# meilisearch/arroy

Measured on NVIDIA H100. Metric: index-build vectors/sec, higher is better.
Workload: dtype f32

## Files before the change

### arroy_b200/csrc/arroy_b200.cu

```cuda
#include <cuda_runtime.h>

#include <algorithm>
#include <atomic>
#include <chrono>
#include <cstdio>
#include <cstdlib>
#include <cstring>
#include <mutex>
#include <stdexcept>
#include <string>
#include <thread>
#include <vector>

#include "../../include/arroy_b200.h"
#include "build.cuh"
#include "search.cuh"
#include <cublas_v2.h>

#include "xrerank.cuh"
#include "tcgemm.cuh"
#include "frerank.cuh"

using namespace ab;

// ... 355 lines not shown
    W.active.ensure(4);
    W.error.ensure(4);
    W.keys.ensure(32ull * tw);
    size_t ws_bytes = (size_t)WS_VECS * ld * 4;
    int use_smem = ws_bytes <= 200 * 1024 ? 1 : 0;
    if (!use_smem) W.scratch.ensure(ws_bytes * tw);
    const int spec = (use_smem && (size_t)WS_VECS_SPEC * ld * 4 <= 200 * 1024 && !(getenv("ARROY_B200_SPEC") && atoi(getenv("ARROY_B200_SPEC")) == 0)) ? 1 : 0;
    if (spec) ws_bytes = (size_t)WS_VECS_SPEC * ld * 4;

    BuildParams P{};
    P.items = c->items.as<float>(); P.ih0 = c->h0.as<float>(); P.ih1 = c->h1.as<float>();
    P.n = (uint32_t)n; P.d = c->dim; P.ld = ld; P.metric = c->metric; P.K = K; P.n_trees = tw;
    P.st = W.st.as<TreeState>(); P.frames = W.frames.as<Frame>(); P.recs = W.recs.as<Record>(); P.rec_cap = rec_cap;
    P.perm[0] = W.perm0.as<uint32_t>(); P.perm[1] = W.perm1.as<uint32_t>();
    P.flags = W.flags.as<uint8_t>(); P.unit_left = W.unit_left.as<uint32_t>(); P.units_per_tree = units;
    P.pool = W.pool.as<float>(); P.pool_stride = pool_stride; P.pool_cap = pool_cap; P.pool_counter = W.pool_counter.as<uint32_t>();
    P.jobs = W.jobs.as<Job>(); P.scratch = W.scratch.as<float>(); P.use_smem_ws = use_smem; P.spec = spec;
    P.active = W.active.as<uint32_t>(); P.error = W.error.as<int32_t>();
    P.sub_rows = nullptr; P.sub_off = nullptr;
    P.lat_mask = getenv("ARROY_B200_LATMASK") ? (uint32_t)atoi(getenv("ARROY_B200_LATMASK")) : 3u;
    P.small_max = getenv("ARROY_B200_SMALL_MAX") ? (uint32_t)atoi(getenv("ARROY_B200_SMALL_MAX")) : (uint32_t)std::max<uint64_t>(2048, (6ull << 20) / (4ull * ld));
    P.max_inner = 1024u;
    P.timing = nullptr;
    if (getenv("ARROY_B200_CTRL_TIMING")) { W.timing.ensure(24 * 8); CK(cudaMemsetAsync(W.timing.p, 0, 24 * 8, c->stream)); P.timing = W.timing.as<unsigned long long>(); }
    if (sub.rows) {
        const uint64_t b = sub.off[t0], e = sub.off[t0 + tw];
        std::vector<uint64_t> off(tw + 1);
        for (uint32_t t = 0; t <= tw; ++t) off[t] = sub.off[t0 + t] - b;
        W.sub_rows.ensure(std::max<size_t>(16, 4ull * (e - b)));
        W.sub_off.ensure(8ull * (tw + 1));
        if (e > b) CK(cudaMemcpyAsync(W.sub_rows.p, sub.rows + b, 4ull * (e - b), cudaMemcpyHostToDevice, c->stream));
        CK(cudaMemcpy(W.sub_off.p, off.data(), 8ull * (tw + 1), cudaMemcpyHostToDevice));
        P.sub_rows = W.sub_rows.as<uint32_t>(); P.sub_off = W.sub_off.as<uint64_t>();
    }

    std::vector<uint32_t> keys((size_t)tw * 8);
    for (uint32_t t = 0; t < tw; ++t)
        for (int i = 0; i < 8; ++i) {
            const uint8_t* s = seeds[t0 + t] + 4 * i;
            keys[(size_t)t * 8 + i] = (uint32_t)s[0] | ((uint32_t)s[1] << 8) | ((uint32_t)s[2] << 16) | ((uint32_t)s[3] << 24);
        }
    CK(cudaMemcpyAsync(W.keys.p, keys.data(), keys.size() * 4, cudaMemcpyHostToDevice, c->stream));
    CK(cudaMemsetAsync(W.pool_counter.p, 0, 4, c->stream));
    CK(cudaMemsetAsync(W.error.p, 0, 4, c->stream));
    CK(cudaMemcpyAsync(W.active.p, &tw, 4, cudaMemcpyHostToDevice, c->stream));
    const uint64_t* d_start = nullptr;
    if (sub.start_pos) {
// ... 66 lines not shown
            P.shadow_small_chunk = getenv("ARROY_B200_SHADOW_CHUNK") ? (uint32_t)std::min(4, std::max(1, atoi(getenv("ARROY_B200_SHADOW_CHUNK")))) : 4u;
            P.shadow_big_units = getenv("ARROY_B200_SHADOW_BIG") ? (uint32_t)atoi(getenv("ARROY_B200_SHADOW_BIG")) : 512u;
            P.shadow_big_chunk = getenv("ARROY_B200_SHADOW_BIGCHUNK") ? (uint32_t)std::max(4, atoi(getenv("ARROY_B200_SHADOW_BIGCHUNK"))) : 8u;
        }
    }
    if (persist) {
        W.slots.ensure(sizeof(PSlot) * tw);
        W.abort.ensure(4);
        CK(cudaMemsetAsync(W.slots.p, 0, sizeof(PSlot) * tw, c->stream));
        CK(cudaMemsetAsync(W.abort.p, 0, 4, c->stream));
        W.cur_normal.ensure(4ull * pool_stride * tw);
        P.slots = W.slots.as<PSlot>();
        P.cur_normal = W.cur_normal.as<float>();
        P.abort = W.abort.as<int>();
        const char* rf = getenv("ARROY_B200_ROOT_FUSE");
        P.root_fused = (!sub.rows && tw >= 2 && P.d >= 32 && (size_t)ROOT_TB * ld * 4 <= psmem && !(rf && atoi(rf) == 0)) ? 1 : 0;
        W.root.ensure(8);
        CK(cudaMemsetAsync(W.root.p, 0, 8, c->stream));
        P.root_ready = W.root.as<uint32_t>(); P.root_ticket = W.root.as<uint32_t>() + 1;
    }

    auto launch_step = [&](cudaStream_t s) {
        launch_control(ctrl1, tw, 1, ctrl_smem, s, P, 0u);
        if (P.planes.hi) work_kernel_shadow<<<c->sm_count * 2, WORK_THREADS, wsmem + perm_smem, s>>>(P.jobs, (int)tw, P.items, P.planes, P.ih0, P.d, P.ld, P.metric, P.shadow_min_units, P.shadow_stats);
        else work_kernel<<<work_grid, WORK_THREADS, wsmem, s>>>(P.jobs, (int)tw, P.items, P.ih0, P.d, P.ld, P.metric, interleave);
    };
    auto launch_tree_step = [&](uint32_t t, cudaStream_t s) {
        launch_control(ctrlc, 1, cluster, ctrl_smem, s, P, t);
        if (P.planes.hi) work_kernel_shadow<<<tree_grid, WORK_THREADS, wsmem1 + perm_smem, s>>>(P.jobs + t, 1, P.items, P.planes, P.ih0, P.d, P.ld, P.metric, P.shadow_min_units, P.shadow_stats);
        else work_kernel<<<tree_grid, WORK_THREADS, wsmem1, s>>>(P.jobs + t, 1, P.items, P.ih0, P.d, P.ld, P.metric, 0);
    };
    if (!lockstep) {
        while (c->tree_streams.size() < tw) { cudaStream_t st; CK(cudaStreamCreateWithFlags(&st, cudaStreamNonBlocking)); c->tree_streams.push_back(st); }
        while (c->tree_events.size() < (size_t)tw + 1) { cudaEvent_t ev; CK(cudaEventCreateWithFlags(&ev, cudaEventDisableTiming)); c->tree_events.push_back(ev); }
    }

    CK(cudaStreamSynchronize(c->stream));
    c->breakdown[0] += ms_since(t_setup);
    auto t_graph = std::chrono::steady_clock::now();
    cudaGraphExec_t gexec = nullptr;
    if (use_graph && !persist) {
        std::vector<uint8_t> key(sizeof(BuildParams) + 16);
        memcpy(key.data(), &P, sizeof(BuildParams));
        int32_t sched[4] = {(lockstep ? 1 : 0) | (interleave << 1) | (cluster << 8), steps_per_batch, (int32_t)tw, (int32_t)ctrl_smem};
        memcpy(key.data() + sizeof(BuildParams), sched, 16);
        if (c->cached_exec && key == c->cached_graph_key) gexec = c->cached_exec;
        else {
            if (c->cached_exec) { cudaGraphExecDestroy(c->cached_exec); c->cached_exec = nullptr; }
            if (c->cached_graph) { cudaGraphDestroy(c->cached_graph); c->cached_graph = nullptr; }
            c->cached_graph_key.clear();
            cudaGraph_t graph = nullptr;
            CK(cudaStreamBeginCapture(c->stream, cudaStreamCaptureModeThreadLocal));
// ... 53 lines not shown
            }
        }
        CK(cudaMemcpyAsync((void*)h_active, W.active.p, 4, cudaMemcpyDeviceToHost, c->stream));
        CK(cudaMemcpyAsync((void*)h_error, W.error.p, 4, cudaMemcpyDeviceToHost, c->stream));
        CK(cudaStreamSynchronize(c->stream));
        steps = 1;
        c->n_launches += 1;
        { float kms = 0; CK(cudaEventElapsedTime(&kms, c->ev_p0, c->ev_p1)); c->stats[5] += kms; }
        if (*h_error != ERR_NONE) {
            const int e = *h_error;
            if (e == ERR_ABORT) throw Cancelled("The corresponding build process has been cancelled");
            if (e == ERR_HANG) throw std::runtime_error("forest build made no progress (persistent schedule watchdog)");
            throw CapacityError(e == ERR_DEPTH ? "tree deeper than MAX_DEPTH frames" : e == ERR_RECORDS ? "node record table overflow" : "normal pool overflow");
        }
        if (*h_active != 0) throw std::runtime_error("forest build ended with unfinished trees (internal state machine error)");
    } else
    for (;;) {
        if (steps > max_steps) throw std::runtime_error("forest build did not converge (internal state machine error)");
        if (use_graph) CK(cudaGraphLaunch(gexec, c->stream));
        else if (profile) {
            for (int i = 0; i < steps_per_batch; ++i) {
                launch_control(ctrl1, tw, 1, ctrl_smem, c->stream, P, 0u);
                CK(cudaEventRecord(pev[2 * i], c->stream));
                if (P.planes.hi) work_kernel_shadow<<<c->sm_count * 2, WORK_THREADS, wsmem + perm_smem, c->stream>>>(P.jobs, (int)tw, P.items, P.planes, P.ih0, P.d, P.ld, P.metric, P.shadow_min_units, P.shadow_stats);
                else work_kernel<<<work_grid, WORK_THREADS, wsmem, c->stream>>>(P.jobs, (int)tw, P.items, P.ih0, P.d, P.ld, P.metric, interleave);
                CK(cudaEventRecord(pev[2 * i + 1], c->stream));
            }
            CK(cudaStreamSynchronize(c->stream));
            for (int i = 0; i < steps_per_batch; ++i) {
                float ms = 0; CK(cudaEventElapsedTime(&ms, pev[2 * i], pev[2 * i + 1])); c->stats[5] += ms;
                if (getenv("ARROY_B200_TRACE") && steps + i < 48) fprintf(stderr, "[trace] step %llu work_kernel %.3f ms\n", (unsigned long long)(steps + i), ms);
            }
        }
        else if (lockstep) { for (int i = 0; i < steps_per_batch; ++i) launch_step(c->stream); CK(cudaGetLastError()); }
        else {
            CK(cudaEventRecord(c->tree_events[0], c->stream));
            for (uint32_t t = 0; t < tw; ++t) {
                cudaStream_t st = c->tree_streams[t];
                CK(cudaStreamWaitEvent(st, c->tree_events[0], 0));
                for (int i = 0; i < steps_per_batch; ++i) launch_tree_step(t, st);
                CK(cudaEventRecord(c->tree_events[1 + t], st));
                CK(cudaStreamWaitEvent(c->stream, c->tree_events[1 + t], 0));
            }
            CK(cudaGetLastError());
        }
        steps += steps_per_batch;
        c->n_launches += 2ull * steps_per_batch * (lockstep ? 1 : tw);
        CK(cudaMemcpyAsync((void*)h_active, W.active.p, 4, cudaMemcpyDeviceToHost, c->stream));
        CK(cudaMemcpyAsync((void*)h_error, W.error.p, 4, cudaMemcpyDeviceToHost, c->stream));
        CK(cudaStreamSynchronize(c->stream));
        if (*h_error != ERR_NONE) {
            int e = *h_error;
            throw CapacityError(e == ERR_DEPTH ? "tree deeper than MAX_DEPTH frames" : e == ERR_RECORDS ? "node record table overflow" : "normal pool overflow");
        }
        if (*h_active == 0) break;
        if (cancel && cancel(cancel_arg)) throw Cancelled("The corresponding build process has been cancelled");
    }
    c->stats[1] += (double)steps;
    c->breakdown[2] += ms_since(t_loop);
    if (P.timing) {
        unsigned long long tv[24]; CK(cudaMemcpy(tv, P.timing, sizeof(tv), cudaMemcpyDeviceToHost));
        const char* nm[20] = {"decide", "rng", "gather", "norms", "two_means_rest", "finish_split", "cluster_scan", "prefix", "partition", "attempts", "inner", "total", "tm_dot_rest", "tm_update", "tm_dots", "tm_finish", "tm_recurrence", "publish_fence", "recur_it0", "recur_it1_9"};
        const double att = (double)std::max<unsigned long long>(tv[9], 1);
        fprintf(stderr, "[ctrl timing] attempts %llu, in-cluster %llu; cycles per attempt:", tv[9], tv[10]);
        for (int i = 0; i < 20; ++i) if (i != 9 && i != 10) fprintf(stderr, " %s %.0f", nm[i], (double)tv[i] / att);
        if (tv[20]) fprintf(stderr, "; fused root pass: %llu cycles on the slowest worker", tv[20]);
        fprintf(stderr, "\n");
    }
    c->breakdown[5] += (double)(steps / steps_per_batch);
    auto t_d2h = std::chrono::steady_clock::now();

    W.final_ids.ensure(4ull * n * tw);
    finalize_kernel<<<dim3(64, tw), 256, 0, c->stream>>>(P, W.final_ids.as<uint32_t>());
    CK(cudaGetLastError());
    std::vector<TreeState> st(tw);
    uint32_t pool_used = 0;
    CK(cudaMemcpyAsync(st.data(), W.st.p, sizeof(TreeState) * tw, cudaMemcpyDeviceToHost, c->stream));
    CK(cudaMemcpyAsync(&pool_used, W.pool_counter.p, 4, cudaMemcpyDeviceToHost, c->stream));
    CK(cudaStreamSynchronize(c->stream));
    if (c->host_waves.size() <= wave_no) c->host_waves.resize(wave_no + 1);
    HostWave& H = c->host_waves[wave_no];
    uint64_t total_recs = 0;
    for (uint32_t t = 0; t < tw; ++t) total_recs += st[t].n_recs;
    H.pool.ensure(std::max<size_t>(16, (size_t)pool_used * pool_stride * 4));
    H.recs.ensure(std::max<size_t>(16, sizeof(Record) * total_recs));
    H.final_rows.ensure(std::max<size_t>(16, 4ull * n * tw));
    if (pool_used) CK(cudaMemcpyAsync(H.pool.p, W.pool.p, (size_t)pool_used * pool_stride * 4, cudaMemcpyDeviceToHost, c->stream));
    CK(cudaMemcpyAsync(H.final_rows.p, W.final_ids.p, 4ull * n * tw, cudaMemcpyDeviceToHost, c->stream));
    out_pool_stride = pool_stride;
// ... 1405 lines not shown
```

### arroy_b200/csrc/build.cuh

```cuda
#pragma once
#include <cooperative_groups.h>
#include "kernels.cuh"

namespace ab {

constexpr int CTRL_THREADS = 256;
constexpr int MAX_DEPTH = 4096;
constexpr uint32_t INLINE_PART_MAX = 8192;
constexpr uint32_t NO_SLOT = 0xffffffffu;

enum : int { PH_START = 0, PH_AWAIT_SCAN = 1, PH_AWAIT_PART = 2, PH_DONE = 3 };
enum : int { REC_DESC = 1, REC_SPLIT = 2 };
enum : int { ERR_NONE = 0, ERR_DEPTH = 1, ERR_RECORDS = 2, ERR_POOL = 3, ERR_HANG = 4, ERR_ABORT = 5 };

struct Frame {
    uint32_t start, len;
    uint32_t left_len;
    uint32_t left_id;
    uint32_t slot;
    uint8_t parity;
    uint8_t stage;
    uint16_t pad;
};

// ... 810 lines not shown
                case 8: proot_units<8>(P, u0, u1, tb, nu0, smN, r_h0, r_cnt); break;
                case 7: proot_units<7>(P, u0, u1, tb, nu0, smN, r_h0, r_cnt); break;
                case 6: proot_units<6>(P, u0, u1, tb, nu0, smN, r_h0, r_cnt); break;
                case 5: proot_units<5>(P, u0, u1, tb, nu0, smN, r_h0, r_cnt); break;
                case 4: proot_units<4>(P, u0, u1, tb, nu0, smN, r_h0, r_cnt); break;
                case 3: proot_units<3>(P, u0, u1, tb, nu0, smN, r_h0, r_cnt); break;
                case 2: proot_units<2>(P, u0, u1, tb, nu0, smN, r_h0, r_cnt); break;
                default: proot_units<1>(P, u0, u1, tb, nu0, smN, r_h0, r_cnt); break;
            }
        }
        __threadfence();
        __syncthreads();
        for (uint32_t t = tid; t < T; t += CTRL_THREADS) atomicAdd(&P.slots[t].done, (unsigned long long)(u1 - u0));
        u0 = nu0;
    }
    if (P.timing != nullptr && tid == 0) atomicMax(P.timing + 20, (unsigned long long)(clock64() - rt0));
}

__device__ __noinline__ void pworker(const BuildParams& P, float* sm_normal) {
    __shared__ uint32_t w_t, w_u0, w_n, w_seq, w_pseq, w_found, w_exit, w_count;
    __shared__ PSlot w_job;
    __shared__ uint32_t w_sm[16];
    __shared__ uint32_t w_list[SCAN_UNIT * PLANES_CHUNK], w_list2[SCAN_UNIT * PLANES_CHUNK];
    __shared__ uint32_t w_cnt[PLANES_CHUNK + 2];
    __shared__ double w_l1[CTRL_THREADS / 32];
    float* sm_perm = sm_normal + P.ld;
    const uint32_t T = P.n_trees;
    const int tid = threadIdx.x, lane = tid & 31, warp = tid >> 5;
    const uint32_t rot = (blockIdx.x - T) * 7u;
    const bool latency_class = ((blockIdx.x - T) & P.lat_mask) == 0u;
    uint32_t loaded_t = 0xffffffffu, loaded_seq = 0xffffffffu;
    float nh0 = 0.f;
    float2 wf = make_float2(0.f, 0.f);
    if (tid == 0) w_exit = 0;
    if (P.root_fused) proot(P, sm_normal);
    for (;;) {
        if (warp == 0) {
            uint32_t found = 0;
            for (uint32_t base = 0; base < T && !found; base += 32) {
                const uint32_t k = base + lane;
                const uint32_t t = k < T ? (rot + k) % T : 0u;
                const unsigned long long tk = k < T ? ld_vol64(&P.slots[t].ticket) : 0ull;
                const bool open_job = k < T && pt_next(tk) < pt_total(tk);
                uint32_t key = !open_job ? 0xffffffffu : (latency_class ? pt_total(tk) : 0x00ffffffu - (pt_total(tk) - pt_next(tk)));
                uint32_t best = key;
#pragma unroll
                for (int o = 16; o > 0; o >>= 1) best = min(best, __shfl_xor_sync(0xffffffffu, best, o));
                if (best != 0xffffffffu) {
                    const unsigned m = __ballot_sync(0xffffffffu, key == best);
                    const int src = __ffs((int)m) - 1;
                    if (lane == src) { w_t = t; w_pseq = pt_seq(tk); }
                    found = 1;
                }
            }
            if (lane == 0) {
                w_found = found;
                if (!found) {
                    if (ld_vol32(P.active) == 0u || *reinterpret_cast<volatile int32_t*>(P.error) != ERR_NONE) w_exit = 1;
                    else __nanosleep(60);
                }
            }
        }
        __syncthreads();
        if (w_exit) return;
        if (!w_found) { __syncthreads(); continue; }
        const uint32_t t = w_t;
        PSlot& sl = P.slots[t];
        const float* nsrc = P.cur_normal + (size_t)t * P.pool_stride;
        const bool want_normal = !(loaded_t == t && loaded_seq == w_pseq);
        float nreg[8];
#pragma unroll
        for (int u = 0; u < 8; ++u) nreg[u] = 0.f;
        if (want_normal) {
#pragma unroll
            for (int u = 0; u < 8; ++u) { const uint32_t i = tid + u * CTRL_THREADS; if (i < P.ld) nreg[u] = __ldcg(nsrc + NORMAL_HDR + i); }
        }
        if (tid == 0) {
            const unsigned long long r = atomicAdd(&sl.ticket, 1ull);
            const uint4 f0 = __ldcg(reinterpret_cast<const uint4*>(&sl) + 1), f1 = __ldcg(reinterpret_cast<const uint4*>(&sl) + 2), f2 = __ldcg(reinterpret_cast<const uint4*>(&sl) + 3);
            uint4* wj = reinterpret_cast<uint4*>(&w_job);
            wj[1] = f0; wj[2] = f1; wj[3] = f2;
            w_seq = pt_seq(r);
            w_u0 = pt_next(r);
            w_n = pt_next(r) < pt_total(r) ? 1u : 0u;
        }
        __syncthreads();
        const uint32_t seq = w_seq, g0 = w_u0;
// ... 7 lines not shown
        if (have) {
            Job jb;
            jb.kind = (int)w_job.kind; jb.len = w_job.len; jb.rows = w_job.rows; jb.normal = nullptr; jb.flags = w_job.flags; jb.margins = nullptr;
            jb.unit_left = w_job.unit_left; jb.dst = w_job.dst; jb.total_left = w_job.total_left; jb.pad = 0;
            const uint32_t chunk = max(1u, w_job.chunk);
            if (jb.kind == JOB_SCAN) {
                const uint32_t units = (jb.len + SCAN_UNIT - 1) / SCAN_UNIT;
                if (want_normal || seq != w_pseq) {
                    double l1 = 0.0;
#pragma unroll
                    for (int u = 0; u < 8; ++u) {
                        const uint32_t i = tid + u * CTRL_THREADS;
                        if (i < P.ld) {
                            sm_normal[i] = nreg[u];
                            if (P.planes.hi != nullptr) { sm_perm[planes_perm_index(i)] = nreg[u]; l1 += (double)fabsf(nreg[u]); }
                        }
                    }
                    if (P.planes.hi != nullptr) { l1 = warp_sum_f64(l1); if (lane == 0) w_l1[warp] = l1; }
                    nh0 = __ldcg(nsrc);
                    loaded_t = t; loaded_seq = seq;
                    __syncthreads();
                    if (P.planes.hi != nullptr) wf = planes_job_factors(w_l1, P.d);
                }
                if (P.planes.hi != nullptr && units > P.shadow_min_units)
                    for (uint32_t u = g0 * chunk; u < min(units, (g0 + 1u) * chunk); u += PLANES_CHUNK)
                        scan_claim_planes(jb, u, min(min(units, (g0 + 1u) * chunk), u + PLANES_CHUNK), P.items, P.planes, P.ih0, P.d, P.ld, P.metric, sm_normal, sm_perm, nh0,
                                          wf.x, wf.y, w_list, w_list2, w_cnt, P.shadow_stats);
                else
                    for (uint32_t u = g0 * chunk; u < min(units, (g0 + 1u) * chunk); ++u) scan_unit<true>(jb, u, P.items, P.ih0, P.d, P.ld, P.metric, sm_normal, nh0, &w_count);
            } else if (jb.kind == JOB_PARTITION) {
                const uint32_t units = (jb.len + PART_UNIT - 1) / PART_UNIT;
                for (uint32_t u = g0 * chunk; u < min(units, (g0 + 1u) * chunk); ++u)
                    partition_block(jb.rows, jb.flags, jb.dst, u * PART_UNIT, jb.len, __ldcg(jb.unit_left + u * (PART_UNIT / SCAN_UNIT)), jb.total_left, w_sm);
            }
            __threadfence();
            __syncthreads();
            if (tid == 0) atomicAdd(&sl.done, 1ull);
        }
        __syncthreads();
    }
}

template <int CS>
__device__ __forceinline__ void cluster_scan_share(const BuildParams& P, const Job& jb, float* sm_normal, uint32_t* sm_count, unsigned rank) {
    for (uint32_t i = threadIdx.x; i < P.ld; i += blockDim.x) sm_normal[i] = jb.normal[NORMAL_HDR + i];
    const float nh0 = jb.normal[0];
    __syncthreads();
    const uint32_t units = (jb.len + SCAN_UNIT - 1) / SCAN_UNIT;
    for (uint32_t u = rank; u < units; u += CS) scan_unit(jb, u, P.items, P.ih0, P.d, P.ld, P.metric, sm_normal, nh0, sm_count);
}

template <bool SMEM_WS, int CS, int METRIC>
__global__ void __launch_bounds__(CTRL_THREADS, (CS == 0 ? 2 : 1)) control_kernel(BuildParams P, uint32_t tree_base) {
    static_assert(CS <= 1 || SMEM_WS, "the cluster path keeps the normal in the shared-memory workspace");
    constexpr bool PERSIST = CS == 0;
    constexpr int CSD = CS < 1 ? 1 : CS;
    extern __shared__ __align__(16) unsigned char ctrl_smem[];
    if (PERSIST && blockIdx.x >= P.n_trees) { pworker(P, reinterpret_cast<float*>(ctrl_smem)); return; }
    __shared__ uint32_t s_scan_count;
    __shared__ TwoMeansShared TM;
// ... 302 lines not shown
```

### arroy_b200/csrc/kernels.cuh

```cuda
#pragma once
#include "exact.cuh"

namespace ab {

constexpr int WORK_THREADS = 256;
constexpr int SCAN_UNIT = 64;
constexpr int PART_UNIT = 256;

enum : int { JOB_NONE = 0, JOB_SCAN = 1, JOB_PARTITION = 2 };

constexpr int NORMAL_HDR = 4;

struct Job {
    int32_t kind;
    uint32_t len;
    const uint32_t* rows;
    const float* normal;
    uint8_t* flags;
    float* margins;
    uint32_t* unit_left;
    uint32_t* dst;
    uint32_t total_left;
    uint32_t pad;
};
// ... 166 lines not shown
    }
}
__device__ __forceinline__ void planes_fma16x2(const uint4 vh, const uint4 vl, const float4 (&y)[4], float& m0, float& m1, float& a0, float& a1) {
    const uint32_t wh[4] = {vh.x ^ 0x80808080u, vh.y ^ 0x80808080u, vh.z ^ 0x80808080u, vh.w ^ 0x80808080u};
    const uint32_t wl[4] = {vl.x ^ 0x80808080u, vl.y ^ 0x80808080u, vl.z ^ 0x80808080u, vl.w ^ 0x80808080u};
#pragma unroll
    for (int j = 0; j < 4; ++j) {
        const float n4[4] = {y[j].x, y[j].y, y[j].z, y[j].w};
#pragma unroll
        for (int k = 0; k < 4; ++k) {
            const float v = fmaf(s8_to_f32(wh[j], (uint32_t)k), 254.0f, s8_to_f32(wl[j], (uint32_t)k));
            if (k & 1) { m1 = fmaf(v, n4[k], m1); a1 = fmaf(fabsf(v), fabsf(n4[k]), a1); }
            else { m0 = fmaf(v, n4[k], m0); a0 = fmaf(fabsf(v), fabsf(n4[k]), a0); }
        }
    }
}

__device__ __forceinline__ float prefilter_finish(int metric, float v, float nh0, float item_h0) {
    if (metric == COSINE) return v;
    if (metric == DOT_PRODUCT) return __fadd_rn(v, __fmul_rn(nh0, item_h0));
    return __fadd_rn(nh0, v);
}

__device__ __forceinline__ void scan_claim_planes(const Job& jb, uint32_t u0, uint32_t u1, const float* __restrict__ items, const PlaneRows pl,
                                                  const float* __restrict__ ih0, uint32_t d, uint32_t ld, int metric, const float* sm_normal, const float* sm_perm,
                                                  float nh0, float w1, float w2, uint32_t* sm_list, uint32_t* sm_list2, uint32_t* sm_cnt, unsigned long long* stats) {
    const int tid = threadIdx.x, lane = tid & 31, warp = tid >> 5, g8 = lane & 7, grp = lane >> 3;
    if (tid <= (int)PLANES_CHUNK + 1) sm_cnt[tid] = 0;
    __syncthreads();
    const uint32_t base = u0 * SCAN_UNIT, end = min(jb.len, u1 * SCAN_UNIT);
    const uint32_t nq = ld >> 4;
    const int nsteps = (int)((nq + 7) >> 3);
    const float4* PN = reinterpret_cast<const float4*>(sm_perm);
    for (uint32_t pbase = base; pbase < end; pbase += 128) {
        uint32_t pos[4], rid[4];
        const uint4* S[4];
#pragma unroll
        for (int r = 0; r < 4; ++r) {
            pos[r] = pbase + warp * 16 + grp * 4 + r;
            rid[r] = pos[r] < end ? (jb.rows ? __ldcg(jb.rows + pos[r]) : pos[r]) : 0u;
            S[r] = reinterpret_cast<const uint4*>(pl.hi + (size_t)rid[r] * ld) + g8;
        }
        float m0[4], m1[4];
#pragma unroll
        for (int r = 0; r < 4; ++r) { m0[r] = 0.f; m1[r] = 0.f; }
        for (int c0 = 0; c0 < nsteps; c0 += 3) {
            uint4 v[3][4];
#pragma unroll
            for (int sidx = 0; sidx < 3; ++sidx)
#pragma unroll
                for (int r = 0; r < 4; ++r) {
                    const uint32_t q = (uint32_t)(c0 + sidx) * 8u + (uint32_t)g8;
                    v[sidx][r] = q < nq ? ldg_stream_u4(S[r] + (c0 + sidx) * 8) : make_uint4(0u, 0u, 0u, 0u);
                }
#pragma unroll
            for (int sidx = 0; sidx < 3; ++sidx) {
                const uint32_t q = (uint32_t)(c0 + sidx) * 8u + (uint32_t)g8;
                float4 y[4];
#pragma unroll
                for (int j = 0; j < 4; ++j) y[j] = q < nq ? PN[(c0 + sidx) * 32 + j * 8 + g8] : make_float4(0.f, 0.f, 0.f, 0.f);
#pragma unroll
                for (int r = 0; r < 4; ++r) planes_fma16(v[sidx][r], y, m0[r], m1[r]);
            }
        }
#pragma unroll
        for (int r = 0; r < 4; ++r) {
            float t = m0[r] + m1[r];
#pragma unroll
            for (int o = 1; o < 8; o <<= 1) t += __shfl_xor_sync(0xffffffffu, t, o);
            const bool valid = pos[r] < end;
            const float s = valid ? __ldg(pl.scale + rid[r]) : 0.f;
            const float mt = prefilter_finish(metric, __fmul_rn(s, t), nh0, (metric == DOT_PRODUCT && valid) ? ih0[rid[r]] : 0.f);
            const bool certain = fabsf(mt) > __fmul_rn(s, w1);
            const bool leader = g8 == 0 && valid;
            const int side = mt > 0.f ? 1 : 0;
            if (leader && certain) jb.flags[pos[r]] = (uint8_t)side;
            if (leader && !certain) sm_list[atomicAdd(&sm_cnt[PLANES_CHUNK], 1u)] = pos[r];
            const unsigned lefts = __ballot_sync(0xffffffffu, leader && certain && side == 0);
            if (lane == 0 && lefts) atomicAdd(&sm_cnt[(pbase + warp * 16 - base) / SCAN_UNIT], (uint32_t)__popc(lefts));
        }
    }
    __syncthreads();
    const uint32_t n1 = sm_cnt[PLANES_CHUNK];
    const float rel2 = planes_rel2(d);
    for (uint32_t it = 0; it * 32u < n1; ++it) {
        const uint32_t idx = it * 32u + (uint32_t)(warp * 4 + grp);
        const bool act = idx < n1;
        const uint32_t p = act ? sm_list[idx] : base;
        const uint32_t r = jb.rows ? __ldcg(jb.rows + p) : p;
        const uint4* Hr = reinterpret_cast<const uint4*>(pl.hi + (size_t)r * ld) + g8;
        const uint4* Lr = reinterpret_cast<const uint4*>(pl.lo + (size_t)r * ld) + g8;
        float m0 = 0.f, m1 = 0.f, a0 = 0.f, a1 = 0.f;
        for (int c0 = 0; c0 < nsteps; c0 += 3) {
            uint4 vh[3], vl[3];
#pragma unroll
            for (int sidx = 0; sidx < 3; ++sidx) {
                const uint32_t q = (uint32_t)(c0 + sidx) * 8u + (uint32_t)g8;
                vh[sidx] = q < nq ? ldg_stream_u4(Hr + (c0 + sidx) * 8) : make_uint4(0u, 0u, 0u, 0u);
                vl[sidx] = q < nq ? ldg_stream_u4(Lr + (c0 + sidx) * 8) : make_uint4(0u, 0u, 0u, 0u);
            }
#pragma unroll
            for (int sidx = 0; sidx < 3; ++sidx) {
                const uint32_t q = (uint32_t)(c0 + sidx) * 8u + (uint32_t)g8;
                float4 y[4];
#pragma unroll
                for (int j = 0; j < 4; ++j) y[j] = q < nq ? PN[(c0 + sidx) * 32 + j * 8 + g8] : make_float4(0.f, 0.f, 0.f, 0.f);
                planes_fma16x2(vh[sidx], vl[sidx], y, m0, m1, a0, a1);
            }
        }
        float m = m0 + m1, a = a0 + a1;
#pragma unroll
        for (int o = 1; o < 8; o <<= 1) { m += __shfl_xor_sync(0xffffffffu, m, o); a += __shfl_xor_sync(0xffffffffu, a, o); }
        const float s2 = __fdiv_rn(__ldg(pl.scale + r), 254.0f);
        const float mt = prefilter_finish(metric, __fmul_rn(s2, m), nh0, (metric == DOT_PRODUCT) ? ih0[r] : 0.f);
        const bool certain = fabsf(mt) > __fmul_rn(s2, __fadd_rn(w2, __fmul_rn(rel2, a)));
        const int side = mt > 0.f ? 1 : 0;
        if (act && g8 == 0) {
            if (certain) { jb.flags[p] = (uint8_t)side; if (side == 0) atomicAdd(&sm_cnt[(p - base) / SCAN_UNIT], 1u); }
            else sm_list2[atomicAdd(&sm_cnt[PLANES_CHUNK + 1], 1u)] = p;
        }
    }
    __syncthreads();
    const uint32_t nl = sm_cnt[PLANES_CHUNK + 1];
    if (stats != nullptr && tid == 0) {
        atomicAdd(stats, (unsigned long long)(end - base));
        if (nl) atomicAdd(stats + 1, (unsigned long long)nl);
        if (n1) atomicAdd(stats + 2, (unsigned long long)n1);
    }
    const int nch = (int)(d >> 5);
    const float4* N = reinterpret_cast<const float4*>(sm_normal);
    for (uint32_t it = 0; it * 32u < nl; ++it) {
        const uint32_t idx = it * 32u + (uint32_t)(warp * 4 + grp);
        const bool act = idx < nl;
        const uint32_t p = act ? sm_list2[idx] : base;
        const uint32_t r = jb.rows ? __ldcg(jb.rows + p) : p;
        const float4* A = reinterpret_cast<const float4*>(items + (size_t)r * ld);
        float4 acc = make_float4(0.f, 0.f, 0.f, 0.f);
        int c = 0;
        for (; c + 8 <= nch; c += 8) {
            float4 x[8];
#pragma unroll
            for (int u = 0; u < 8; ++u) x[u] = ldg_stream(A + (c + u) * 8 + g8);
#pragma unroll
            for (int u = 0; u < 8; ++u) {
                const float4 y = N[(c + u) * 8 + g8];
                acc.x = fmaf(x[u].x, y.x, acc.x); acc.y = fmaf(x[u].y, y.y, acc.y); acc.z = fmaf(x[u].z, y.z, acc.z); acc.w = fmaf(x[u].w, y.w, acc.w);
            }
        }
        for (; c < nch; ++c) {
            const float4 x = ldg_stream(A + c * 8 + g8), y = N[c * 8 + g8];
            acc.x = fmaf(x.x, y.x, acc.x); acc.y = fmaf(x.y, y.y, acc.y); acc.z = fmaf(x.z, y.z, acc.z); acc.w = fmaf(x.w, y.w, acc.w);
        }
        float da = group8_hsum(acc);
        const float* row = items + (size_t)r * ld;
        for (uint32_t i = (uint32_t)nch * 32u; i < d; ++i) da = __fadd_rn(da, __fmul_rn(row[i], sm_normal[i]));
        const int sa = side_of(margin_finish(metric, da, nh0, (metric == DOT_PRODUCT) ? ih0[r] : 0.f));
        if (act && g8 == 0) { jb.flags[p] = (uint8_t)sa; if (sa == 0) atomicAdd(&sm_cnt[(p - base) / SCAN_UNIT], 1u); }
    }
    __syncthreads();
    if (tid < (int)(u1 - u0)) jb.unit_left[u0 + tid] = sm_cnt[tid];
}

__device__ __forceinline__ float2 planes_job_factors(const double* sm_l1, uint32_t d) {
    double s = 0.0;
#pragma unroll
    for (int w = 0; w < 8; ++w) s += sm_l1[w];
    s *= 1.0 + 0x1p-30;
    return make_float2(__double2float_ru(s * (double)planes_k1(d)), __double2float_ru(s * (double)planes_w2(d)));
}
__device__ __forceinline__ double warp_sum_f64(double v) {
#pragma unroll
    for (int o = 16; o > 0; o >>= 1) v += __shfl_xor_sync(0xffffffffu, v, o);
    return v;
}

__device__ __forceinline__ void partition_block(const uint32_t* __restrict__ src, const uint8_t* __restrict__ flags, uint32_t* __restrict__ dst,
                                                uint32_t base, uint32_t len, uint32_t left_before, uint32_t total_left, uint32_t* sm_w) {
    const int lane = threadIdx.x & 31, warp = threadIdx.x >> 5;
    uint32_t p = base + threadIdx.x;
    bool valid = p < len;
    int f = valid ? (int)__ldcg(flags + p) : 1;
    uint32_t id = valid ? __ldcg(src + p) : 0;
// ... 68 lines not shown
    for (uint32_t u = blockIdx.x; u < total; u += gridDim.x) {
        int lo = 0, hi = njobs;
        while (hi - lo > 1) { int mid = (lo + hi) >> 1; if (sm_prefix[mid] <= u) lo = mid; else hi = mid; }
        const int j = lo;
        const Job jb = jobs[j];
        const uint32_t unit = u - sm_prefix[j];
        if (jb.kind == JOB_SCAN) {
            if (loaded_job != j) {
                __syncthreads();
                for (uint32_t i = threadIdx.x; i < ld; i += blockDim.x) sm_normal[i] = jb.normal[NORMAL_HDR + i];
                nh0 = jb.normal[0];
                loaded_job = j;
                __syncthreads();
            }
            scan_unit(jb, unit, items, ih0, d, ld, metric, sm_normal, nh0, &sm_count);
        } else {
            partition_block(jb.rows, jb.flags, jb.dst, unit * PART_UNIT, jb.len, jb.unit_left[unit * (PART_UNIT / SCAN_UNIT)], jb.total_left, sm_w);
        }
    }
}

__global__ void __launch_bounds__(WORK_THREADS, 2)
work_kernel_shadow(const Job* __restrict__ jobs, int njobs, const float* __restrict__ items, const PlaneRows planes, const float* __restrict__ ih0,
                   uint32_t d, uint32_t ld, int metric, uint32_t min_units, unsigned long long* stats) {
    extern __shared__ __align__(16) unsigned char smem_raw[];
    float* sm_normal = reinterpret_cast<float*>(smem_raw);
    float* sm_perm = sm_normal + ld;
    uint32_t* sm_prefix = reinterpret_cast<uint32_t*>(sm_perm + planes_perm_floats(ld));
    __shared__ uint32_t sm_count;
    __shared__ uint32_t sm_w[16];
    __shared__ uint32_t sm_list[SCAN_UNIT * PLANES_CHUNK], sm_list2[SCAN_UNIT * PLANES_CHUNK];
    __shared__ uint32_t sm_cnt[PLANES_CHUNK + 2];
    __shared__ double sm_l1[WORK_THREADS / 32];
    auto via_shadow = [&](const Job& jb) { return jb.kind == JOB_SCAN && jb.margins == nullptr && (jb.len + SCAN_UNIT - 1) / SCAN_UNIT > min_units; };
    for (int j = threadIdx.x; j < njobs; j += blockDim.x) {
        const Job jb = jobs[j];
        const uint32_t units = (jb.len + SCAN_UNIT - 1) / SCAN_UNIT;
        sm_prefix[j] = jb.kind == JOB_SCAN ? (via_shadow(jb) ? (units + PLANES_CHUNK - 1) / PLANES_CHUNK : units) : (jb.kind == JOB_PARTITION ? (jb.len + PART_UNIT - 1) / PART_UNIT : 0u);
    }
    __syncthreads();
    if (threadIdx.x < 32) {
        const int per = (njobs + 31) / 32;
        const int b = threadIdx.x * per, e = min(b + per, njobs);
        uint32_t loc = 0;
        for (int i = b; i < e; ++i) loc += sm_prefix[i];
        uint32_t inc = loc;
        for (int o = 1; o < 32; o <<= 1) { uint32_t y = __shfl_up_sync(0xffffffffu, inc, o); if ((int)threadIdx.x >= o) inc += y; }
        uint32_t run = inc - loc;
        for (int i = b; i < e; ++i) { uint32_t x = sm_prefix[i]; sm_prefix[i] = run; run += x; }
        if (threadIdx.x == 31) sm_prefix[njobs] = inc;
    }
    __syncthreads();
    const uint32_t total = sm_prefix[njobs];
    int loaded_job = -1;
    float nh0 = 0.f;
    float2 wf = make_float2(0.f, 0.f);
    for (uint32_t u = blockIdx.x; u < total; u += gridDim.x) {
        int lo = 0, hi = njobs;
        while (hi - lo > 1) { int mid = (lo + hi) >> 1; if (sm_prefix[mid] <= u) lo = mid; else hi = mid; }
        const int j = lo;
        const Job jb = jobs[j];
        const uint32_t item = u - sm_prefix[j];
        if (jb.kind == JOB_SCAN) {
            if (loaded_job != j) {
                __syncthreads();
                double l1 = 0.0;
                for (uint32_t i = threadIdx.x; i < ld; i += blockDim.x) {
                    const float v = jb.normal[NORMAL_HDR + i];
                    sm_normal[i] = v;
                    sm_perm[planes_perm_index(i)] = v;
                    l1 += (double)fabsf(v);
                }
                l1 = warp_sum_f64(l1);
                if ((threadIdx.x & 31) == 0) sm_l1[threadIdx.x >> 5] = l1;
                nh0 = jb.normal[0];
                loaded_job = j;
                __syncthreads();
                wf = planes_job_factors(sm_l1, d);
            }
            if (via_shadow(jb)) {
                const uint32_t units = (jb.len + SCAN_UNIT - 1) / SCAN_UNIT;
                scan_claim_planes(jb, item * PLANES_CHUNK, min(units, (item + 1u) * PLANES_CHUNK), items, planes, ih0, d, ld, metric, sm_normal, sm_perm, nh0, wf.x, wf.y,
                                  sm_list, sm_list2, sm_cnt, stats);
            } else scan_unit<true>(jb, item, items, ih0, d, ld, metric, sm_normal, nh0, &sm_count);
        } else {
            partition_block(jb.rows, jb.flags, jb.dst, item * PART_UNIT, jb.len, jb.unit_left[item * (PART_UNIT / SCAN_UNIT)], jb.total_left, sm_w);
        }
    }
}

__global__ void __launch_bounds__(256) norms_kernel(const float* __restrict__ items, uint64_t n, uint32_t d, uint32_t ld, float* __restrict__ out, uint32_t* max_bits) {
    const int lane = threadIdx.x & 31;
    uint64_t warp_global = (uint64_t)blockIdx.x * (blockDim.x >> 5) + (threadIdx.x >> 5);
    uint64_t nwarps = (uint64_t)gridDim.x * (blockDim.x >> 5);
    for (uint64_t r0 = warp_global * 4; r0 < n; r0 += nwarps * 4) {
        float res;
        if (d >= 32) {
            const int g8 = lane & 7, grp = lane >> 3;
            uint64_t r = r0 + grp;
            bool v = r < n;
            const float4* A = reinterpret_cast<const float4*>(items + (size_t)(v ? r : 0) * ld);
            float4 acc = make_float4(0.f, 0.f, 0.f, 0.f);
            const int nch = d >> 5;
#pragma unroll 4
            for (int c = 0; c < nch; ++c) {
                float4 x = ldg_stream(A + c * 8 + g8);
                acc.x = fmaf(x.x, x.x, acc.x); acc.y = fmaf(x.y, x.y, acc.y); acc.z = fmaf(x.z, x.z, acc.z); acc.w = fmaf(x.w, x.w, acc.w);
            }
            float dt = group8_hsum(acc);
            const float* row = items + (size_t)(v ? r : 0) * ld;
            for (uint32_t i = nch * 32; i < d; ++i) dt = __fadd_rn(dt, __fmul_rn(row[i], row[i]));
// ... 268 lines not shown
```

Baseline: 3.904 million.

## Stage row ids in shared memory and prefetch plane rows into L2 in shadow scan

The shadow-plane prefilter scan now loads each chunk's row ids once into a shared array, and the later stages reuse them instead of re-reading the global rows index. The persistent worker issues bulk L2 prefetches of the high-plane rows up front, and of low-plane rows for uncertain items as they are queued. Scale loads are hoisted ahead of the dot loop, and the stage-2 unroll is doubled from 3 to 6. Compile-time-gated per-stage cycle timing for scanners is also added. The cost is extra shared memory and register pressure, plus possibly wasted prefetch bandwidth.

```diff
diff --git a/arroy_b200/csrc/arroy_b200.cu b/arroy_b200/csrc/arroy_b200.cu
--- a/arroy_b200/csrc/arroy_b200.cu
+++ b/arroy_b200/csrc/arroy_b200.cu
@@ -401,7 +401,7 @@
     P.small_max = getenv("ARROY_B200_SMALL_MAX") ? (uint32_t)atoi(getenv("ARROY_B200_SMALL_MAX")) : (uint32_t)std::max<uint64_t>(2048, (6ull << 20) / (4ull * ld));
     P.max_inner = 1024u;
     P.timing = nullptr;
-    if (getenv("ARROY_B200_CTRL_TIMING")) { W.timing.ensure(24 * 8); CK(cudaMemsetAsync(W.timing.p, 0, 24 * 8, c->stream)); P.timing = W.timing.as<unsigned long long>(); }
+    if (getenv("ARROY_B200_CTRL_TIMING")) { W.timing.ensure(TIMING_SLOTS * 8); CK(cudaMemsetAsync(W.timing.p, 0, TIMING_SLOTS * 8, c->stream)); P.timing = W.timing.as<unsigned long long>(); }
     if (sub.rows) {
         const uint64_t b = sub.off[t0], e = sub.off[t0 + tw];
         std::vector<uint64_t> off(tw + 1);
@@ -514,12 +514,12 @@
 
     auto launch_step = [&](cudaStream_t s) {
         launch_control(ctrl1, tw, 1, ctrl_smem, s, P, 0u);
-        if (P.planes.hi) work_kernel_shadow<<<c->sm_count * 2, WORK_THREADS, wsmem + perm_smem, s>>>(P.jobs, (int)tw, P.items, P.planes, P.ih0, P.d, P.ld, P.metric, P.shadow_min_units, P.shadow_stats);
+        if (P.planes.hi) work_kernel_shadow<<<c->sm_count * 2, WORK_THREADS, wsmem + perm_smem, s>>>(P.jobs, (int)tw, P.items, P.planes, P.ih0, P.d, P.ld, P.metric, P.shadow_min_units, P.shadow_stats WT_DO(, P.timing));
         else work_kernel<<<work_grid, WORK_THREADS, wsmem, s>>>(P.jobs, (int)tw, P.items, P.ih0, P.d, P.ld, P.metric, interleave);
     };
     auto launch_tree_step = [&](uint32_t t, cudaStream_t s) {
         launch_control(ctrlc, 1, cluster, ctrl_smem, s, P, t);
-        if (P.planes.hi) work_kernel_shadow<<<tree_grid, WORK_THREADS, wsmem1 + perm_smem, s>>>(P.jobs + t, 1, P.items, P.planes, P.ih0, P.d, P.ld, P.metric, P.shadow_min_units, P.shadow_stats);
+        if (P.planes.hi) work_kernel_shadow<<<tree_grid, WORK_THREADS, wsmem1 + perm_smem, s>>>(P.jobs + t, 1, P.items, P.planes, P.ih0, P.d, P.ld, P.metric, P.shadow_min_units, P.shadow_stats WT_DO(, P.timing));
         else work_kernel<<<tree_grid, WORK_THREADS, wsmem1, s>>>(P.jobs + t, 1, P.items, P.ih0, P.d, P.ld, P.metric, 0);
     };
     if (!lockstep) {
@@ -619,7 +619,7 @@
             for (int i = 0; i < steps_per_batch; ++i) {
                 launch_control(ctrl1, tw, 1, ctrl_smem, c->stream, P, 0u);
                 CK(cudaEventRecord(pev[2 * i], c->stream));
-                if (P.planes.hi) work_kernel_shadow<<<c->sm_count * 2, WORK_THREADS, wsmem + perm_smem, c->stream>>>(P.jobs, (int)tw, P.items, P.planes, P.ih0, P.d, P.ld, P.metric, P.shadow_min_units, P.shadow_stats);
+                if (P.planes.hi) work_kernel_shadow<<<c->sm_count * 2, WORK_THREADS, wsmem + perm_smem, c->stream>>>(P.jobs, (int)tw, P.items, P.planes, P.ih0, P.d, P.ld, P.metric, P.shadow_min_units, P.shadow_stats WT_DO(, P.timing));
                 else work_kernel<<<work_grid, WORK_THREADS, wsmem, c->stream>>>(P.jobs, (int)tw, P.items, P.ih0, P.d, P.ld, P.metric, interleave);
                 CK(cudaEventRecord(pev[2 * i + 1], c->stream));
             }
@@ -656,12 +656,16 @@
     c->stats[1] += (double)steps;
     c->breakdown[2] += ms_since(t_loop);
     if (P.timing) {
-        unsigned long long tv[24]; CK(cudaMemcpy(tv, P.timing, sizeof(tv), cudaMemcpyDeviceToHost));
+        unsigned long long tv[TIMING_SLOTS]; CK(cudaMemcpy(tv, P.timing, sizeof(tv), cudaMemcpyDeviceToHost));
         const char* nm[20] = {"decide", "rng", "gather", "norms", "two_means_rest", "finish_split", "cluster_scan", "prefix", "partition", "attempts", "inner", "total", "tm_dot_rest", "tm_update", "tm_dots", "tm_finish", "tm_recurrence", "publish_fence", "recur_it0", "recur_it1_9"};
         const double att = (double)std::max<unsigned long long>(tv[9], 1);
         fprintf(stderr, "[ctrl timing] attempts %llu, in-cluster %llu; cycles per attempt:", tv[9], tv[10]);
         for (int i = 0; i < 20; ++i) if (i != 9 && i != 10) fprintf(stderr, " %s %.0f", nm[i], (double)tv[i] / att);
         if (tv[20]) fprintf(stderr, "; fused root pass: %llu cycles on the slowest worker", tv[20]);
+        const unsigned long long* wt = tv + WT_SLOT0;
+        const double cl = (double)std::max<unsigned long long>(wt[WT_CLAIMS], 1);
+        if (WT_COMPILED) fprintf(stderr, "; scanners: %llu pre-filter claims, cycles per claim: poll_idle %.0f claim %.0f stage1 %.0f stage2 %.0f stage3 %.0f report %.0f other_jobs %.0f",
+                wt[WT_CLAIMS], wt[WT_POLL] / cl, wt[WT_CLAIM] / cl, wt[WT_S1] / cl, wt[WT_S2] / cl, wt[WT_S3] / cl, wt[WT_REPORT] / cl, wt[WT_OTHER] / cl);
         fprintf(stderr, "\n");
     }
     c->breakdown[5] += (double)(steps / steps_per_batch);
diff --git a/arroy_b200/csrc/build.cuh b/arroy_b200/csrc/build.cuh
--- a/arroy_b200/csrc/build.cuh
+++ b/arroy_b200/csrc/build.cuh
@@ -856,8 +856,10 @@
     __shared__ PSlot w_job;
     __shared__ uint32_t w_sm[16];
     __shared__ uint32_t w_list[SCAN_UNIT * PLANES_CHUNK], w_list2[SCAN_UNIT * PLANES_CHUNK];
+    __shared__ uint32_t w_rid[SCAN_UNIT * PLANES_CHUNK];
     __shared__ uint32_t w_cnt[PLANES_CHUNK + 2];
     __shared__ double w_l1[CTRL_THREADS / 32];
+    WT_DO(__shared__ long long tm[WT_N + 1]; const bool timed = P.timing != nullptr;)
     float* sm_perm = sm_normal + P.ld;
     const uint32_t T = P.n_trees;
     const int tid = threadIdx.x, lane = tid & 31, warp = tid >> 5;
@@ -868,6 +870,7 @@
     float2 wf = make_float2(0.f, 0.f);
     if (tid == 0) w_exit = 0;
     if (P.root_fused) proot(P, sm_normal);
+    WT_DO(if (timed && tid == 0) { for (int i = 0; i < WT_N; ++i) tm[i] = 0; tm[WT_N] = clock64(); })
     for (;;) {
         if (warp == 0) {
             uint32_t found = 0;
@@ -896,7 +899,9 @@
             }
         }
         __syncthreads();
+        WT_DO(if (w_exit && timed && tid == 0) { WT_ADD(WT_POLL); for (int i = 0; i < WT_N; ++i) atomicAdd(P.timing + WT_SLOT0 + i, (unsigned long long)tm[i]); })
         if (w_exit) return;
+        WT_ADD(WT_POLL);
         if (!w_found) { __syncthreads(); continue; }
         const uint32_t t = w_t;
         PSlot& sl = P.slots[t];
@@ -950,20 +955,25 @@
                     __syncthreads();
                     if (P.planes.hi != nullptr) wf = planes_job_factors(w_l1, P.d);
                 }
+                WT_ADD(WT_CLAIM);
+                WT_DO(if (timed && tid == 0 && P.planes.hi != nullptr && units > P.shadow_min_units) tm[WT_CLAIMS] += 1;)
                 if (P.planes.hi != nullptr && units > P.shadow_min_units)
                     for (uint32_t u = g0 * chunk; u < min(units, (g0 + 1u) * chunk); u += PLANES_CHUNK)
                         scan_claim_planes(jb, u, min(min(units, (g0 + 1u) * chunk), u + PLANES_CHUNK), P.items, P.planes, P.ih0, P.d, P.ld, P.metric, sm_normal, sm_perm, nh0,
-                                          wf.x, wf.y, w_list, w_list2, w_cnt, P.shadow_stats);
+                                          wf.x, wf.y, w_list, w_list2, w_rid, w_cnt, P.shadow_stats, true WT_DO(, timed, tm));
                 else
                     for (uint32_t u = g0 * chunk; u < min(units, (g0 + 1u) * chunk); ++u) scan_unit<true>(jb, u, P.items, P.ih0, P.d, P.ld, P.metric, sm_normal, nh0, &w_count);
             } else if (jb.kind == JOB_PARTITION) {
+                WT_ADD(WT_CLAIM);
                 const uint32_t units = (jb.len + PART_UNIT - 1) / PART_UNIT;
                 for (uint32_t u = g0 * chunk; u < min(units, (g0 + 1u) * chunk); ++u)
                     partition_block(jb.rows, jb.flags, jb.dst, u * PART_UNIT, jb.len, __ldcg(jb.unit_left + u * (PART_UNIT / SCAN_UNIT)), jb.total_left, w_sm);
             }
+            WT_ADD(WT_OTHER);
             __threadfence();
             __syncthreads();
             if (tid == 0) atomicAdd(&sl.done, 1ull);
+            WT_ADD(WT_REPORT);
         }
         __syncthreads();
     }
diff --git a/arroy_b200/csrc/kernels.cuh b/arroy_b200/csrc/kernels.cuh
--- a/arroy_b200/csrc/kernels.cuh
+++ b/arroy_b200/csrc/kernels.cuh
@@ -212,13 +212,31 @@
     return __fadd_rn(nh0, v);
 }
 
+enum { WT_CLAIMS = 0, WT_POLL = 1, WT_CLAIM = 2, WT_S1 = 3, WT_S2 = 4, WT_S3 = 5, WT_REPORT = 6, WT_OTHER = 7, WT_N = 8 };
+constexpr int WT_SLOT0 = 21;
+constexpr int TIMING_SLOTS = WT_SLOT0 + WT_N;
+#ifdef ARROY_B200_WORKER_TIMING
+constexpr bool WT_COMPILED = true;
+#define WT_DO(...) __VA_ARGS__
+#else
+constexpr bool WT_COMPILED = false;
+#define WT_DO(...)
+#endif
+#define WT_ADD(id_) WT_DO(do { if (timed && threadIdx.x == 0) { const long long now_ = clock64(); tm[id_] += now_ - tm[WT_N]; tm[WT_N] = now_; } } while (0))
+
 __device__ __forceinline__ void scan_claim_planes(const Job& jb, uint32_t u0, uint32_t u1, const float* __restrict__ items, const PlaneRows pl,
                                                   const float* __restrict__ ih0, uint32_t d, uint32_t ld, int metric, const float* sm_normal, const float* sm_perm,
-                                                  float nh0, float w1, float w2, uint32_t* sm_list, uint32_t* sm_list2, uint32_t* sm_cnt, unsigned long long* stats) {
+                                                  float nh0, float w1, float w2, uint32_t* sm_list, uint32_t* sm_list2, uint32_t* sm_rid, uint32_t* sm_cnt,
+                                                  unsigned long long* stats, bool prefetch_hi WT_DO(, bool timed, long long* tm)) {
     const int tid = threadIdx.x, lane = tid & 31, warp = tid >> 5, g8 = lane & 7, grp = lane >> 3;
+    const uint32_t base = u0 * SCAN_UNIT, end = min(jb.len, u1 * SCAN_UNIT);
     if (tid <= (int)PLANES_CHUNK + 1) sm_cnt[tid] = 0;
-    __syncthreads();
-    const uint32_t base = u0 * SCAN_UNIT, end = min(jb.len, u1 * SCAN_UNIT);
+    if ((uint32_t)tid < end - base) {
+        const uint32_t r = jb.rows ? __ldcg(jb.rows + base + tid) : base + tid;
+        sm_rid[tid] = r;
+        if (prefetch_hi) asm volatile("cp.async.bulk.prefetch.L2.global [%0], %1;" ::"l"(pl.hi + (size_t)r * ld), "r"(ld) : "memory");
+    }
+    __syncthreads();
     const uint32_t nq = ld >> 4;
     const int nsteps = (int)((nq + 7) >> 3);
     const float4* PN = reinterpret_cast<const float4*>(sm_perm);
@@ -228,9 +246,12 @@
 #pragma unroll
         for (int r = 0; r < 4; ++r) {
             pos[r] = pbase + warp * 16 + grp * 4 + r;
-            rid[r] = pos[r] < end ? (jb.rows ? __ldcg(jb.rows + pos[r]) : pos[r]) : 0u;
+            rid[r] = pos[r] < end ? sm_rid[pos[r] - base] : 0u;
             S[r] = reinterpret_cast<const uint4*>(pl.hi + (size_t)rid[r] * ld) + g8;
         }
+        float sc[4];
+#pragma unroll
+        for (int r = 0; r < 4; ++r) sc[r] = pos[r] < end ? __ldg(pl.scale + rid[r]) : 0.f;
         float m0[4], m1[4];
 #pragma unroll
         for (int r = 0; r < 4; ++r) { m0[r] = 0.f; m1[r] = 0.f; }
@@ -259,38 +280,43 @@
 #pragma unroll
             for (int o = 1; o < 8; o <<= 1) t += __shfl_xor_sync(0xffffffffu, t, o);
             const bool valid = pos[r] < end;
-            const float s = valid ? __ldg(pl.scale + rid[r]) : 0.f;
+            const float s = sc[r];
             const float mt = prefilter_finish(metric, __fmul_rn(s, t), nh0, (metric == DOT_PRODUCT && valid) ? ih0[rid[r]] : 0.f);
             const bool certain = fabsf(mt) > __fmul_rn(s, w1);
             const bool leader = g8 == 0 && valid;
             const int side = mt > 0.f ? 1 : 0;
             if (leader && certain) jb.flags[pos[r]] = (uint8_t)side;
-            if (leader && !certain) sm_list[atomicAdd(&sm_cnt[PLANES_CHUNK], 1u)] = pos[r];
+            if (leader && !certain) {
+                sm_list[atomicAdd(&sm_cnt[PLANES_CHUNK], 1u)] = pos[r];
+                asm volatile("cp.async.bulk.prefetch.L2.global [%0], %1;" ::"l"(pl.lo + (size_t)rid[r] * ld), "r"(ld) : "memory");
+            }
             const unsigned lefts = __ballot_sync(0xffffffffu, leader && certain && side == 0);
             if (lane == 0 && lefts) atomicAdd(&sm_cnt[(pbase + warp * 16 - base) / SCAN_UNIT], (uint32_t)__popc(lefts));
         }
     }
     __syncthreads();
+    WT_ADD(WT_S1);
     const uint32_t n1 = sm_cnt[PLANES_CHUNK];
     const float rel2 = planes_rel2(d);
     for (uint32_t it = 0; it * 32u < n1; ++it) {
         const uint32_t idx = it * 32u + (uint32_t)(warp * 4 + grp);
         const bool act = idx < n1;
         const uint32_t p = act ? sm_list[idx] : base;
-        const uint32_t r = jb.rows ? __ldcg(jb.rows + p) : p;
+        const uint32_t r = sm_rid[p - base];
+        const float sc = __ldg(pl.scale + r);
         const uint4* Hr = reinterpret_cast<const uint4*>(pl.hi + (size_t)r * ld) + g8;
         const uint4* Lr = reinterpret_cast<const uint4*>(pl.lo + (size_t)r * ld) + g8;
         float m0 = 0.f, m1 = 0.f, a0 = 0.f, a1 = 0.f;
-        for (int c0 = 0; c0 < nsteps; c0 += 3) {
-            uint4 vh[3], vl[3];
-#pragma unroll
-            for (int sidx = 0; sidx < 3; ++sidx) {
+        for (int c0 = 0; c0 < nsteps; c0 += 6) {
+            uint4 vh[6], vl[6];
+#pragma unroll
+            for (int sidx = 0; sidx < 6; ++sidx) {
                 const uint32_t q = (uint32_t)(c0 + sidx) * 8u + (uint32_t)g8;
                 vh[sidx] = q < nq ? ldg_stream_u4(Hr + (c0 + sidx) * 8) : make_uint4(0u, 0u, 0u, 0u);
                 vl[sidx] = q < nq ? ldg_stream_u4(Lr + (c0 + sidx) * 8) : make_uint4(0u, 0u, 0u, 0u);
             }
 #pragma unroll
-            for (int sidx = 0; sidx < 3; ++sidx) {
+            for (int sidx = 0; sidx < 6; ++sidx) {
                 const uint32_t q = (uint32_t)(c0 + sidx) * 8u + (uint32_t)g8;
                 float4 y[4];
 #pragma unroll
@@ -301,7 +327,7 @@
         float m = m0 + m1, a = a0 + a1;
 #pragma unroll
         for (int o = 1; o < 8; o <<= 1) { m += __shfl_xor_sync(0xffffffffu, m, o); a += __shfl_xor_sync(0xffffffffu, a, o); }
-        const float s2 = __fdiv_rn(__ldg(pl.scale + r), 254.0f);
+        const float s2 = __fdiv_rn(sc, 254.0f);
         const float mt = prefilter_finish(metric, __fmul_rn(s2, m), nh0, (metric == DOT_PRODUCT) ? ih0[r] : 0.f);
         const bool certain = fabsf(mt) > __fmul_rn(s2, __fadd_rn(w2, __fmul_rn(rel2, a)));
         const int side = mt > 0.f ? 1 : 0;
@@ -311,6 +337,7 @@
         }
     }
     __syncthreads();
+    WT_ADD(WT_S2);
     const uint32_t nl = sm_cnt[PLANES_CHUNK + 1];
     if (stats != nullptr && tid == 0) {
         atomicAdd(stats, (unsigned long long)(end - base));
@@ -323,7 +350,7 @@
         const uint32_t idx = it * 32u + (uint32_t)(warp * 4 + grp);
         const bool act = idx < nl;
         const uint32_t p = act ? sm_list2[idx] : base;
-        const uint32_t r = jb.rows ? __ldcg(jb.rows + p) : p;
+        const uint32_t r = sm_rid[p - base];
         const float4* A = reinterpret_cast<const float4*>(items + (size_t)r * ld);
         float4 acc = make_float4(0.f, 0.f, 0.f, 0.f);
         int c = 0;
@@ -348,6 +375,7 @@
         if (act && g8 == 0) { jb.flags[p] = (uint8_t)sa; if (sa == 0) atomicAdd(&sm_cnt[(p - base) / SCAN_UNIT], 1u); }
     }
     __syncthreads();
+    WT_ADD(WT_S3);
     if (tid < (int)(u1 - u0)) jb.unit_left[u0 + tid] = sm_cnt[tid];
 }
 
@@ -462,16 +490,19 @@
 
 __global__ void __launch_bounds__(WORK_THREADS, 2)
 work_kernel_shadow(const Job* __restrict__ jobs, int njobs, const float* __restrict__ items, const PlaneRows planes, const float* __restrict__ ih0,
-                   uint32_t d, uint32_t ld, int metric, uint32_t min_units, unsigned long long* stats) {
+                   uint32_t d, uint32_t ld, int metric, uint32_t min_units, unsigned long long* stats WT_DO(, unsigned long long* timing)) {
     extern __shared__ __align__(16) unsigned char smem_raw[];
     float* sm_normal = reinterpret_cast<float*>(smem_raw);
     float* sm_perm = sm_normal + ld;
     uint32_t* sm_prefix = reinterpret_cast<uint32_t*>(sm_perm + planes_perm_floats(ld));
     __shared__ uint32_t sm_count;
     __shared__ uint32_t sm_w[16];
-    __shared__ uint32_t sm_list[SCAN_UNIT * PLANES_CHUNK], sm_list2[SCAN_UNIT * PLANES_CHUNK];
+    __shared__ uint32_t sm_list[SCAN_UNIT * PLANES_CHUNK], sm_list2[SCAN_UNIT * PLANES_CHUNK], sm_rid[SCAN_UNIT * PLANES_CHUNK];
     __shared__ uint32_t sm_cnt[PLANES_CHUNK + 2];
     __shared__ double sm_l1[WORK_THREADS / 32];
+    WT_DO(__shared__ long long tm[WT_N + 1];
+          const bool timed = timing != nullptr;
+          if (timed && threadIdx.x == 0) { for (int i = 0; i < WT_N; ++i) tm[i] = 0; tm[WT_N] = clock64(); })
     auto via_shadow = [&](const Job& jb) { return jb.kind == JOB_SCAN && jb.margins == nullptr && (jb.len + SCAN_UNIT - 1) / SCAN_UNIT > min_units; };
     for (int j = threadIdx.x; j < njobs; j += blockDim.x) {
         const Job jb = jobs[j];
@@ -496,6 +527,7 @@
     float nh0 = 0.f;
     float2 wf = make_float2(0.f, 0.f);
     for (uint32_t u = blockIdx.x; u < total; u += gridDim.x) {
+        WT_ADD(WT_OTHER);
         int lo = 0, hi = njobs;
         while (hi - lo > 1) { int mid = (lo + hi) >> 1; if (sm_prefix[mid] <= u) lo = mid; else hi = mid; }
         const int j = lo;
@@ -519,14 +551,17 @@
                 wf = planes_job_factors(sm_l1, d);
             }
             if (via_shadow(jb)) {
+                WT_ADD(WT_CLAIM);
+                WT_DO(if (timed && threadIdx.x == 0) tm[WT_CLAIMS] += 1;)
                 const uint32_t units = (jb.len + SCAN_UNIT - 1) / SCAN_UNIT;
                 scan_claim_planes(jb, item * PLANES_CHUNK, min(units, (item + 1u) * PLANES_CHUNK), items, planes, ih0, d, ld, metric, sm_normal, sm_perm, nh0, wf.x, wf.y,
-                                  sm_list, sm_list2, sm_cnt, stats);
+                                  sm_list, sm_list2, sm_rid, sm_cnt, stats, false WT_DO(, timed, tm));
             } else scan_unit<true>(jb, item, items, ih0, d, ld, metric, sm_normal, nh0, &sm_count);
         } else {
             partition_block(jb.rows, jb.flags, jb.dst, item * PART_UNIT, jb.len, jb.unit_left[item * (PART_UNIT / SCAN_UNIT)], jb.total_left, sm_w);
         }
     }
+    WT_DO(if (timed && threadIdx.x == 0) { WT_ADD(WT_OTHER); for (int i = 0; i < WT_N; ++i) atomicAdd(timing + WT_SLOT0 + i, (unsigned long long)tm[i]); })
 }
 
 __global__ void __launch_bounds__(256) norms_kernel(const float* __restrict__ items, uint64_t n, uint32_t d, uint32_t ld, float* __restrict__ out, uint32_t* max_bits) {
```

New measurement: 3.963 million, median of 6. 1.5% higher.
